# ModelCloud/GPTQModel

Hardware: NVIDIA H100
Metric: W4A16 g128 QuantLinear: decode tok/s + prefill TFLOPS vs HBM/TC roofline (higher is better)
Workload: dtype f16

## Files before the change

### gptqmodel_b200/csrc/b2q_common.cuh

```cuda
#pragma once
#include <cuda_fp16.h>
#include <cuda_bf16.h>
#include <cuda_runtime.h>
#include <stdint.h>

namespace b2q {

__device__ __forceinline__ uint32_t smem_u32(const void* p) {
  return static_cast<uint32_t>(__cvta_generic_to_shared(p));
}

__device__ __forceinline__ uint4 ldg_nc_v4(const void* p) {
  uint4 r;
  asm volatile("ld.global.nc.L1::no_allocate.v4.u32 {%0,%1,%2,%3}, [%4];"
               : "=r"(r.x), "=r"(r.y), "=r"(r.z), "=r"(r.w)
               : "l"(p));
  return r;
}

__device__ __forceinline__ uint32_t lop3_and_or(uint32_t a, uint32_t mask, uint32_t orv) {
  uint32_t r;
  asm("lop3.b32 %0, %1, %2, %3, 0xEA;" : "=r"(r) : "r"(a), "r"(mask), "r"(orv));
  return r;
}

__device__ __forceinline__ float fhfma_lo(uint32_t a2, uint32_t b2, float c) {
  return fmaf(__low2float(*reinterpret_cast<const __half2*>(&a2)), __low2float(*reinterpret_cast<const __half2*>(&b2)), c);
}
__device__ __forceinline__ float fhfma_hi(uint32_t a2, uint32_t b2, float c) {
  return fmaf(__high2float(*reinterpret_cast<const __half2*>(&a2)), __high2float(*reinterpret_cast<const __half2*>(&b2)),
              c);
}
__device__ __forceinline__ float fbfma_lo(uint32_t a2, uint32_t b2, float c) {
  return fmaf(__uint_as_float(a2 << 16), __uint_as_float(b2 << 16), c);
}
__device__ __forceinline__ float fbfma_hi(uint32_t a2, uint32_t b2, float c) {
  return fmaf(__uint_as_float(a2 & 0xFFFF0000u), __uint_as_float(b2 & 0xFFFF0000u), c);
}

__device__ __forceinline__ void mbar_init(uint32_t bar, uint32_t count) {
  asm volatile("mbarrier.init.shared::cta.b64 [%0], %1;" ::"r"(bar), "r"(count));
}
__device__ __forceinline__ void mbar_expect_tx(uint32_t bar, uint32_t bytes) {
  asm volatile("mbarrier.arrive.expect_tx.shared::cta.b64 _, [%0], %1;" ::"r"(bar), "r"(bytes) : "memory");
}
__device__ __forceinline__ void mbar_expect_tx_only(uint32_t bar, uint32_t bytes) {
  asm volatile("mbarrier.expect_tx.relaxed.cta.shared::cta.b64 [%0], %1;" ::"r"(bar), "r"(bytes) : "memory");
}
__device__ __forceinline__ void mbar_arrive(uint32_t bar) {
  asm volatile("mbarrier.arrive.shared::cta.b64 _, [%0];" ::"r"(bar) : "memory");
}
__device__ __forceinline__ bool mbar_try_wait(uint32_t bar, uint32_t parity) {
  uint32_t ok;
  asm volatile(
      "{ .reg .pred p; mbarrier.try_wait.parity.shared::cta.b64 p, [%1], %2; selp.u32 %0, 1, 0, p; }"
      : "=r"(ok)
      : "r"(bar), "r"(parity)
      : "memory");
  return ok != 0;
}
__device__ __forceinline__ void mbar_wait(uint32_t bar, uint32_t parity) {
  while (!mbar_try_wait(bar, parity)) {
  }
}
__device__ __forceinline__ void fence_mbar_init() {
  asm volatile("fence.mbarrier_init.release.cluster;" ::: "memory");
}
__device__ __forceinline__ void fence_proxy_async_smem() {
  asm volatile("fence.proxy.async.shared::cta;" ::: "memory");
}

__device__ __forceinline__ void tma_load_2d(uint32_t dst, const void* tmap, uint32_t bar, int c0, int c1) {
  asm volatile(
      "cp.async.bulk.tensor.2d.shared::cluster.global.mbarrier::complete_tx::bytes [%0], [%1, {%3, %4}], [%2];"
      ::"r"(dst), "l"(tmap), "r"(bar), "r"(c0), "r"(c1)
      : "memory");
}
__device__ __forceinline__ void bulk_load(uint32_t dst, const void* src, uint32_t bytes, uint32_t bar) {
  asm volatile(
      "cp.async.bulk.shared::cluster.global.mbarrier::complete_tx::bytes [%0], [%1], %2, [%3];"
      ::"r"(dst), "l"(src), "r"(bytes), "r"(bar)
      : "memory");
}
__device__ __forceinline__ void prefetch_tmap(const void* tmap) {
  asm volatile("prefetch.tensormap [%0];" ::"l"(tmap) : "memory");
}

constexpr unsigned long long B2Q_PEER_TIMEOUT_NS = 2000000000ull;
__device__ __forceinline__ bool spin_until_geq_sys(const uint32_t* p, uint32_t target) {
  unsigned long long t0 = 0;
  for (unsigned it = 0;; ++it) {
    uint32_t v;
    asm volatile("ld.acquire.sys.global.u32 %0, [%1];" : "=r"(v) : "l"(p) : "memory");
    if ((int32_t)(v - target) >= 0) return true;
    if ((it & 1023u) == 1023u) {
      unsigned long long now;
      asm volatile("mov.u64 %0, %%globaltimer;" : "=l"(now));
      if (t0 == 0) t0 = now;
      else if (now - t0 > B2Q_PEER_TIMEOUT_NS) return false;
    }
  }
}

__device__ __forceinline__ uint32_t cluster_ctarank() {
  uint32_t r;
  asm volatile("mov.u32 %0, %%cluster_ctarank;" : "=r"(r));
  return r;
}
__device__ __forceinline__ uint32_t cluster_nctarank() {
  uint32_t r;
  asm volatile("mov.u32 %0, %%cluster_nctarank;" : "=r"(r));
  return r;
}
__device__ __forceinline__ void cluster_sync_all() {
  asm volatile("barrier.cluster.arrive.release.aligned;\n\tbarrier.cluster.wait.acquire.aligned;" ::: "memory");
}
__device__ __forceinline__ float ld_dsmem_f32(uint32_t local_saddr, uint32_t cta) {
  uint32_t ra;
  float v;
  asm volatile("mapa.shared::cluster.u32 %0, %1, %2;" : "=r"(ra) : "r"(local_saddr), "r"(cta));
  asm volatile("ld.shared::cluster.f32 %0, [%1];" : "=f"(v) : "r"(ra) : "memory");
  return v;
}
__device__ __forceinline__ void ld_dsmem_v4(uint32_t cluster_saddr, float (&v)[4]) {
  asm volatile("ld.shared::cluster.v4.f32 {%0,%1,%2,%3}, [%4];"
               : "=f"(v[0]), "=f"(v[1]), "=f"(v[2]), "=f"(v[3])
               : "r"(cluster_saddr)
               : "memory");
}
__device__ __forceinline__ void ld_dsmem_v4(uint32_t cluster_saddr, int (&v)[4]) {
  asm volatile("ld.shared::cluster.v4.s32 {%0,%1,%2,%3}, [%4];"
               : "=r"(v[0]), "=r"(v[1]), "=r"(v[2]), "=r"(v[3])
               : "r"(cluster_saddr)
               : "memory");
}
template <int NCH, bool FROM_ZERO, typename V>
__device__ __forceinline__ void dsmem_sum4(uint32_t local, uint32_t stride, uint32_t nrank, V (&a)[NCH][4]) {
  if (FROM_ZERO) {
#pragma unroll
    for (int c = 0; c < NCH; ++c)
#pragma unroll
      for (int i = 0; i < 4; ++i) a[c][i] = V(0);
  }
  for (uint32_t r = 0; r < nrank; ++r) {
    uint32_t ra;
    asm volatile("mapa.shared::cluster.u32 %0, %1, %2;" : "=r"(ra) : "r"(local), "r"(r));
#pragma unroll
    for (int c = 0; c < NCH; ++c) {
      V v[4];
      ld_dsmem_v4(ra + c * stride, v);
#pragma unroll
      for (int i = 0; i < 4; ++i) a[c][i] = (FROM_ZERO || r != 0) ? a[c][i] + v[i] : v[i];
    }
  }
}

template <typename T>
struct ET;
template <>
struct ET<__half> {
  static constexpr int FMT = 0;
  static constexpr uint32_t MAGIC = 0x64006400u;
  static constexpr float LO_BASE = 1024.f;
  static constexpr float HI_BASE = 64.f;
  static constexpr float HI_SCALE = 0.0625f;
  __device__ static __forceinline__ void unpack_w4(uint32_t w, uint32_t (&h)[4]) {
    h[0] = lop3_and_or(w, 0x000f000fu, MAGIC);
    h[1] = lop3_and_or(w, 0x00f000f0u, MAGIC);
    const uint32_t w8 = w >> 8;
    h[2] = lop3_and_or(w8, 0x000f000fu, MAGIC);
    h[3] = lop3_and_or(w8, 0x00f000f0u, MAGIC);
  }
  __device__ static __forceinline__ float to_f(__half v) { return __half2float(v); }
  __device__ static __forceinline__ __half from_f(float v) { return __float2half_rn(v); }
  __device__ static __forceinline__ float fma_lo(uint32_t a, uint32_t b, float c) { return fhfma_lo(a, b, c); }
  __device__ static __forceinline__ float fma_hi(uint32_t a, uint32_t b, float c) { return fhfma_hi(a, b, c); }
  __device__ static __forceinline__ uint32_t pack2(float a, float b) {
    __half2 h = __floats2half2_rn(a, b);
    return *reinterpret_cast<uint32_t*>(&h);
  }
};
template <>
struct ET<__nv_bfloat16> {
  static constexpr int FMT = 1;
  static constexpr uint32_t MAGIC = 0x43004300u;
  static constexpr float LO_BASE = 128.f;
  static constexpr float HI_BASE = 128.f;
  static constexpr float HI_SCALE = 1.0f;
  __device__ static __forceinline__ void unpack_w4(uint32_t w, uint32_t (&h)[4]) {
    h[0] = lop3_and_or(w, 0x000f000fu, MAGIC);
    h[1] = lop3_and_or(w >> 4, 0x000f000fu, MAGIC);
    h[2] = lop3_and_or(w >> 8, 0x000f000fu, MAGIC);
    h[3] = lop3_and_or(w >> 12, 0x000f000fu, MAGIC);
  }
  __device__ static __forceinline__ float to_f(__nv_bfloat16 v) { return __bfloat162float(v); }
  __device__ static __forceinline__ __nv_bfloat16 from_f(float v) { return __float2bfloat16_rn(v); }
  __device__ static __forceinline__ float fma_lo(uint32_t a, uint32_t b, float c) { return fbfma_lo(a, b, c); }
  __device__ static __forceinline__ float fma_hi(uint32_t a, uint32_t b, float c) { return fbfma_hi(a, b, c); }
  __device__ static __forceinline__ uint32_t pack2(float a, float b) {
    __nv_bfloat162 h = __floats2bfloat162_rn(a, b);
    return *reinterpret_cast<uint32_t*>(&h);
  }
};

__device__ __forceinline__ uint32_t e4m3x2(float lo, float hi) {
  uint16_t r;
  asm("cvt.rn.satfinite.e4m3x2.f32 %0, %1, %2;" : "=h"(r) : "f"(hi), "f"(lo));
  return r;
}
template <typename T>
__device__ __forceinline__ uint2 fblk_code8(const uint4& v, float s) {
  const T* h = reinterpret_cast<const T*>(&v);
  float q[8];
#pragma unroll
  for (int e = 0; e < 8; ++e) q[e] = ET<T>::to_f(h[e]) / s;
  return make_uint2(e4m3x2(q[0], q[1]) | (e4m3x2(q[2], q[3]) << 16), e4m3x2(q[4], q[5]) | (e4m3x2(q[6], q[7]) << 16));
}

}
```

### gptqmodel_b200/csrc/b2q_gemm.cu

```cuda
#include <cuda.h>

#include "b2q_common.cuh"
#include "b2q_dequant.cuh"
#include "b2q_gemm.cuh"
#include "b2q_internal.h"
#include "b2q_wgmma.cuh"

namespace b2q {

template <typename T, int BITS, bool ASYM, int STAGES, bool FP8 = false>
__global__ void __launch_bounds__(G_THREADS, 1)
    gemm_kernel(const __grid_constant__ CUtensorMap tmap_x, const __grid_constant__ GemmSets S, int M, int K,
                int gshc) {
  using C = GemmCfg<BITS, STAGES>;
  using E = ET<T>;
  extern __shared__ uint8_t smem_raw[];
  const uint32_t smem_base = (smem_u32(smem_raw) + 1023u) & ~1023u;
  uint8_t* smem = smem_raw + (smem_base - smem_u32(smem_raw));

  const uint32_t sA = smem_base;
  const uint32_t sB = sA + STAGES * C::A_BYTES;
  const uint32_t sP = sB + STAGES * C::B_BYTES;
  const uint32_t sBar = sP + STAGES * C::P_BYTES;
  const uint32_t bar_full = sBar, bar_bready = sBar + 8 * STAGES, bar_empty = sBar + 16 * STAGES;

  int set = 0, tn = blockIdx.x;
  if (S.nsets > 1 && tn >= S.tn_end[0]) {
    set = (S.nsets > 2 && tn >= S.tn_end[1]) ? 2 : 1;
    tn -= S.tn_end[set - 1];
  }
  const int N = S.N[set];
  const uint4* __restrict__ packed = S.packed[set];
  const T* __restrict__ scales = reinterpret_cast<const T*>(S.scales[set]);
  const uint32_t* __restrict__ qzeros = S.qzeros[set];

  const int warp = threadIdx.x >> 5, lane = threadIdx.x & 31;
  const int NT = N >> 5;
  const int n0 = tn * G_BN, m0 = blockIdx.y * G_BM;
  const int nt0 = n0 >> 5;
  const int ntiles = min(4, NT - nt0);
  const int nkb = K / G_BK;

  if (threadIdx.x == 0) {
    prefetch_tmap(&tmap_x);
    for (int s = 0; s < STAGES; ++s) {
      mbar_init(bar_full + 8 * s, 1);
      mbar_init(bar_bready + 8 * s, G_DQ_THREADS);
      mbar_init(bar_empty + 8 * s, 1);
    }
    fence_mbar_init();
  }
  __syncthreads();

  if (warp == 8) {
    if (lane == 0) {
      const int FT = N >> 4, ft0 = n0 >> 4;
      const uint32_t pbytes4 = (uint32_t)min(8, FT - ft0) * 512u;
      const uint32_t pbytes8 = (uint32_t)ntiles * C::SUB * 512u;
      for (int kb = 0; kb < nkb; ++kb) {
        const int s = kb % STAGES;
        const uint32_t ph = (kb / STAGES) & 1;
        mbar_wait(bar_empty + 8 * s, ph ^ 1);
        const int g0 = (2 * kb) >> gshc, g1 = (2 * kb + 1) >> gshc;
        const int nrows = (g1 != g0) ? 2 : 1;
        const uint32_t sbytes = (uint32_t)min(G_BN, N - n0) * 2u, zbytes = ASYM ? sbytes / 4u : 0u;
        mbar_expect_tx(bar_full + 8 * s,
                       C::A_BYTES + (BITS == 4 ? pbytes4 + nrows * (sbytes + zbytes) : 2 * pbytes8));
        tma_load_2d(sA + s * C::A_BYTES, &tmap_x, bar_full + 8 * s, kb * G_BK, m0);
        if (BITS == 4) {
          bulk_load(sP + s * C::P_BYTES, packed + ((size_t)kb * FT + ft0) * 32, pbytes4, bar_full + 8 * s);
          for (int r = 0; r < nrows; ++r) {
            const int gr = r ? g1 : g0;
            bulk_load(sP + s * C::P_BYTES + 4096 + r * 320, scales + (size_t)gr * N + n0, sbytes, bar_full + 8 * s);
            if (ASYM)
              bulk_load(sP + s * C::P_BYTES + 4096 + r * 320 + 256, qzeros + (size_t)gr * (N >> 3) + (n0 >> 3),
                        zbytes, bar_full + 8 * s);
          }
        } else {
#pragma unroll
          for (int j = 0; j < 2; ++j)
            bulk_load(sP + s * C::P_BYTES + j * C::P_CHUNK_BYTES,
                      packed + ((size_t)(kb * 2 + j) * NT + nt0) * C::SUB * 32, pbytes8, bar_full + 8 * s);
        }
      }
    }
  } else if (warp < 4) {
    float acc[2][G_BN / 2];
#pragma unroll
    for (int mb = 0; mb < 2; ++mb)
#pragma unroll
      for (int i = 0; i < G_BN / 2; ++i) acc[mb][i] = 0.f;
    for (int kb = 0; kb < nkb; ++kb) {
      const int s = kb % STAGES;
      const uint32_t ph = (kb / STAGES) & 1;
      mbar_wait(bar_full + 8 * s, ph);
      mbar_wait(bar_bready + 8 * s, ph);
      wgmma_fence();
      const uint64_t bdesc = wgmma_desc_k_sw128(sB + s * C::B_BYTES);
      const uint64_t adesc = wgmma_desc_k_sw128(sA + s * C::A_BYTES);
#pragma unroll
      for (int k = 0; k < G_BK / 16; ++k) {
#pragma unroll
        for (int mb = 0; mb < 2; ++mb)
          Wgmma<E::FMT, G_BN>::mma(acc[mb], adesc + 512 * mb + 2 * k, bdesc + 2 * k, (kb | k) != 0 ? 1u : 0u);
      }
      wgmma_commit();
      wgmma_wait<1>();
      if (kb > 0 && threadIdx.x == 0) mbar_arrive(bar_empty + 8 * ((kb - 1) % STAGES));
    }
    wgmma_wait<0>();
#pragma unroll
    for (int mb = 0; mb < 2; ++mb) wgmma_fence_regs(acc[mb]);

    const T* __restrict__ bias = reinterpret_cast<const T*>(S.bias[set]);
    T* __restrict__ out = reinterpret_cast<T*>(S.out[set]);
#pragma unroll
    for (int mb = 0; mb < 2; ++mb) {
#pragma unroll
      for (int h = 0; h < 2; ++h) {
        const int row = m0 + 64 * mb + 16 * warp + (lane >> 2) + 8 * h;
        if (row >= M) continue;
        T* dst = out + (size_t)row * N;
#pragma unroll
        for (int j = 0; j < G_BN / 8; ++j) {
          const int col = n0 + 8 * j + 2 * (lane & 3);
          if (col >= N) continue;
          float f0 = acc[mb][4 * j + 2 * h], f1 = acc[mb][4 * j + 2 * h + 1];
          if (bias != nullptr) {
            f0 = E::to_f(E::from_f(f0)) + E::to_f(bias[col]);
            f1 = E::to_f(E::from_f(f1)) + E::to_f(bias[col + 1]);
          }
          *reinterpret_cast<uint32_t*>(dst + col) = E::pack2(f0, f1);
        }
      }
    }
  } else {
    const int t = threadIdx.x - G_MMA_THREADS;
    constexpr int PF = 32 / BITS;
    constexpr int ZSYM = 1 << (BITS - 1);
    if (BITS == 4) {
      const int lp = t & 31, g = lp >> 2, tt = lp & 3;
      int f[4];
      f[0] = (t >> 5) * 16 + g;
      f[1] = f[0] + 8;
      f[2] = f[0] + 64;
      f[3] = f[0] + 72;
      for (int kb = 0; kb < nkb; ++kb) {
        const int s = kb % STAGES;
        const uint32_t ph = (kb / STAGES) & 1;
        mbar_wait(bar_full + 8 * s, ph);
        const uint8_t* pst = smem + (sP - smem_base) + s * C::P_BYTES;
        const uint4* pj = reinterpret_cast<const uint4*>(pst);
        const int grow = ((2 * kb + (tt >> 1)) >> gshc) - ((2 * kb) >> gshc);
        const uint8_t* srow = pst + 4096 + grow * 320;
#pragma unroll
        for (int u = 0; u < 2; ++u) {
          const uint4 pv = pj[t + u * 128];
          const uint32_t s_lo = *reinterpret_cast<const uint16_t*>(srow + f[2 * u] * 2);
          const uint32_t s_hi = *reinterpret_cast<const uint16_t*>(srow + f[2 * u + 1] * 2);
          int zl = ZSYM, zh = ZSYM;
          if (ASYM) {
            const uint32_t zwl = *reinterpret_cast<const uint32_t*>(srow + 256 + (f[2 * u] >> 3) * 4);
            const uint32_t zwh = *reinterpret_cast<const uint32_t*>(srow + 256 + (f[2 * u + 1] >> 3) * 4);
            zl = (int)((zwl >> (4 * g)) & 15u);
            zh = (int)((zwh >> (4 * g)) & 15u);
          }
          uint4 lo[2], hi[2];
          Dequant<T, 4>::run(pv, s_lo, zl, s_hi, zh, lo, hi);
          const uint32_t sw = (uint32_t)g;
          const uint32_t rlo = sB + s * C::B_BYTES + f[2 * u] * 128;
          const uint32_t rhi = rlo + 8 * 128;
#pragma unroll
          for (int c = 0; c < 2; ++c) {
            const uint32_t off = (((uint32_t)(2 * tt + c)) ^ sw) << 4;
            asm volatile("st.shared.v4.u32 [%0], {%1,%2,%3,%4};" ::"r"(rlo + off), "r"(lo[c].x), "r"(lo[c].y),
                         "r"(lo[c].z), "r"(lo[c].w)
                         : "memory");
            asm volatile("st.shared.v4.u32 [%0], {%1,%2,%3,%4};" ::"r"(rhi + off), "r"(hi[c].x), "r"(hi[c].y),
                         "r"(hi[c].z), "r"(hi[c].w)
                         : "memory");
          }
        }
        fence_proxy_async_smem();
        mbar_arrive(bar_bready + 8 * s);
      }
    } else {
      const int n = n0 + t;
      const int nsafe = (n < N) ? n : 0;
      const int ntl = t >> 5;
      SZRaw cur[2], nxt[2];
      cur[0] = load_sz<T, BITS, ASYM>(scales, qzeros, 0, nsafe, N);
      cur[1] = load_sz<T, BITS, ASYM>(scales, qzeros, 1 >> gshc, nsafe, N);
      for (int kb = 0; kb < nkb; ++kb) {
        const int s = kb % STAGES;
        const uint32_t ph = (kb / STAGES) & 1;
        if (kb + 1 < nkb) {
          nxt[0] = load_sz<T, BITS, ASYM>(scales, qzeros, (2 * kb + 2) >> gshc, nsafe, N);
          nxt[1] = load_sz<T, BITS, ASYM>(scales, qzeros, (2 * kb + 3) >> gshc, nsafe, N);
        }
        mbar_wait(bar_full + 8 * s, ph);
        const uint32_t brow = sB + s * C::B_BYTES + t * 128;
        const uint32_t sw = (uint32_t)(t & 7);
#pragma unroll
        for (int j = 0; j < 2; ++j) {
          int z = ZSYM;
          if (ASYM) z = (int)((cur[j].zw >> (BITS * (nsafe % PF))) & ((1u << BITS) - 1));
          Fp8Div dv = {};
          if constexpr (FP8) dv = fp8_div_of<T>(cur[j].s);
          const uint4* pj = reinterpret_cast<const uint4*>(smem + (sP - smem_base) + s * C::P_BYTES +
                                                           j * C::P_CHUNK_BYTES);
#pragma unroll
          for (int h = 0; h < 2; ++h) {
            const uint4 pv = pj[(ntl * 2 + h) * 32 + lane];
            uint4 o[2];
            if constexpr (FP8)
              DequantFp8<T>::run(pv, dv, o);
            else
              Dequant<T, 8>::run(pv, cur[j].s, z, o);
#pragma unroll
            for (int c = 0; c < 2; ++c) {
              const uint32_t addr = brow + (((uint32_t)(j * 4 + h * 2 + c) ^ sw) << 4);
              asm volatile("st.shared.v4.u32 [%0], {%1,%2,%3,%4};" ::"r"(addr), "r"(o[c].x), "r"(o[c].y),
                           "r"(o[c].z), "r"(o[c].w)
                           : "memory");
            }
          }
        }
        fence_proxy_async_smem();
        mbar_arrive(bar_bready + 8 * s);
        cur[0] = nxt[0];
        cur[1] = nxt[1];
      }
    }
  }
}

typedef CUresult (*EncodeTiledFn)(CUtensorMap*, CUtensorMapDataType, cuuint32_t, void*, const cuuint64_t*,
                                  const cuuint64_t*, const cuuint32_t*, const cuuint32_t*, CUtensorMapInterleave,
                                  CUtensorMapSwizzle, CUtensorMapL2promotion, CUtensorMapFloatOOBfill);

int make_tmap_2d(CUtensorMap* map, CUtensorMapDataType dt, const void* p, int dim0, int dim1, size_t stride, int box0,
                 int box1, CUtensorMapSwizzle sw) {
  struct Entry {
    const void* p;
    int dt, dim0, dim1, box0, box1, sw;
    size_t stride;
    CUtensorMap map;
  };
  constexpr int NCACHE = 64;
  static thread_local Entry cache[NCACHE];
  static thread_local int next = 0, filled = 0;
  for (int i = 0; i < filled; ++i) {
    const Entry& c = cache[i];
    if (c.p == p && c.dt == (int)dt && c.dim0 == dim0 && c.dim1 == dim1 && c.stride == stride && c.box0 == box0 &&
        c.box1 == box1 && c.sw == (int)sw) {
      *map = c.map;
      return 0;
    }
  }
  static EncodeTiledFn enc = nullptr;
  if (enc == nullptr) {
    void* f = nullptr;
    cudaDriverEntryPointQueryResult qres;
    if (cudaGetDriverEntryPoint("cuTensorMapEncodeTiled", &f, cudaEnableDefault, &qres) == cudaSuccess &&
        qres == cudaDriverEntryPointSuccess)
      enc = reinterpret_cast<EncodeTiledFn>(f);
  }
  if (enc == nullptr) {
    set_error("b2q: cuTensorMapEncodeTiled not available from the driver");
    return -1;
  }
  cuuint64_t gdim[2] = {(cuuint64_t)dim0, (cuuint64_t)dim1};
  cuuint64_t gstride[1] = {(cuuint64_t)stride};
  cuuint32_t boxd[2] = {(cuuint32_t)box0, (cuuint32_t)box1};
  cuuint32_t estr[2] = {1, 1};
  CUresult r = enc(map, dt, 2, const_cast<void*>(p), gdim, gstride, boxd, estr, CU_TENSOR_MAP_INTERLEAVE_NONE, sw,
                   CU_TENSOR_MAP_L2_PROMOTION_L2_256B, CU_TENSOR_MAP_FLOAT_OOB_FILL_NONE);
  if (r != CUDA_SUCCESS) {
    set_error("b2q: cuTensorMapEncodeTiled failed (%d) for %p [%d, %d] box [%d, %d]", (int)r, p, dim1, dim0, box1, box0);
    return -1;
  }
  cache[next] = {p, (int)dt, dim0, dim1, box0, box1, (int)sw, stride, *map};
  next = (next + 1) % NCACHE;
  if (filled < NCACHE) ++filled;
  return 0;
}

int gemm_gshc(const MmArgs& a) {
  if (a.group_size == 32) return 0;
  if (a.group_size == 64) return 1;
  if (a.group_size == 128) return 2;
  return 31;
}


template <typename T, int BITS, bool ASYM, int STAGES, bool FP8 = false>
static int launch_gemm_t(const MmArgs& a, const void* x, const GemmSets& S) {
  using C = GemmCfg<BITS, STAGES>;
  CUtensorMap tmap;
  if (make_tmap_2d(&tmap, a.dtype == 0 ? CU_TENSOR_MAP_DATA_TYPE_FLOAT16 : CU_TENSOR_MAP_DATA_TYPE_BFLOAT16, x, a.K, a.M,
                   (size_t)a.K * 2, G_BK, G_BM, CU_TENSOR_MAP_SWIZZLE_128B) != 0)
    return -1;
  auto kern = gemm_kernel<T, BITS, ASYM, STAGES, FP8>;
  static int smem_opted[32] = {};
  if (int e = ensure_dyn_smem(kern, C::SMEM_BYTES, smem_opted, "b2q_gemm")) return e;
  dim3 grid(S.tn_end[S.nsets - 1], (a.M + G_BM - 1) / G_BM, 1);
  kern<<<grid, G_THREADS, C::SMEM_BYTES, a.stream>>>(tmap, S, a.M, a.K, gemm_gshc(a));
  return (int)cudaGetLastError();
}

static int launch_gemm_sets(const MmArgs& a, const void* x, const GemmSets& S) {
  if (a.fp8) return a.dtype == 0 ? launch_gemm_t<__half, 8, false, 4, true>(a, x, S)
                                 : launch_gemm_t<__nv_bfloat16, 8, false, 4, true>(a, x, S);
  const bool asym = S.qzeros[0] != nullptr;
#define B2Q_GEMM_CASE(T, BITS, ST) \
  (asym ? launch_gemm_t<T, BITS, true, ST>(a, x, S) : launch_gemm_t<T, BITS, false, ST>(a, x, S))
  if (a.dtype == 0) return a.bits == 4 ? B2Q_GEMM_CASE(__half, 4, 4) : B2Q_GEMM_CASE(__half, 8, 4);
  return a.bits == 4 ? B2Q_GEMM_CASE(__nv_bfloat16, 4, 4) : B2Q_GEMM_CASE(__nv_bfloat16, 8, 4);
#undef B2Q_GEMM_CASE
}

int launch_gemm_multi(const MmArgs& a, const void* x, int nsets, const void* const* packed, const void* const* scales,
                      const int32_t* const* qzeros, const void* const* bias, void* const* out, const int* Ns) {
  GemmSets S = {};
  S.nsets = nsets;
  int tn = 0;
  for (int i = 0; i < nsets; ++i) {
    tn += (Ns[i] + G_BN - 1) / G_BN;
    S.tn_end[i] = tn;
    S.N[i] = Ns[i];
    S.packed[i] = (const uint4*)packed[i];
    S.scales[i] = scales[i];
    S.qzeros[i] = (const uint32_t*)qzeros[i];
    S.bias[i] = bias[i];
    S.out[i] = out[i];
  }
  for (int i = nsets; i < G_MAX_SETS; ++i) S.tn_end[i] = tn;
  return launch_gemm_sets(a, x, S);
}

int launch_gemm(const MmArgs& a) {
  if (a.K % G_BK != 0) {
    set_error("b2q_gemm: K=%d must be a multiple of %d", a.K, G_BK);
    return -1;
  }
  const void* x = a.x;
  if (a.perm != nullptr) {
    const size_t need = (size_t)a.M * a.K * 2;
    if (a.workspace == nullptr || a.workspace_bytes < need) {
      set_error("b2q_gemm: act-order needs a %zu-byte workspace (got %zu)", need, a.workspace_bytes);
      return -1;
    }
    int e = launch_permute_cols(a.x, a.perm, a.workspace, a.M, a.K, a.stream);
    if (e != 0) return e;
    x = a.workspace;
  }
  if (a.M <= 128 && env().midm && midm_supported(a)) return launch_midm(a, x);
  const void* packed = a.packed;
  const void* scales = a.scales;
  const int32_t* qzeros = (const int32_t*)a.qzeros;
  const void* bias = a.bias;
  void* out = a.out;
  return launch_gemm_multi(a, x, 1, &packed, &scales, &qzeros, &bias, &out, &a.N);
}

}
```

### gptqmodel_b200/csrc/b2q_gemm.cuh

```cuda
#pragma once
#include "b2q_common.cuh"

namespace b2q {

constexpr int G_BM = 128;
constexpr int G_BN = 128;
constexpr int G_BK = 64;
constexpr int G_MMA_THREADS = 128;
constexpr int G_DQ_THREADS = 128;
constexpr int G_THREADS = G_MMA_THREADS + G_DQ_THREADS + 32;

template <int BITS, int STAGES>
struct GemmCfg {
  static constexpr int SUB = BITS / 4;
  static constexpr int A_BYTES = G_BM * G_BK * 2;
  static constexpr int B_BYTES = G_BN * G_BK * 2;
  static constexpr int P_CHUNK_BYTES = 4 * SUB * 512;
  static constexpr int P_BYTES = 2 * P_CHUNK_BYTES + (BITS == 4 ? 1024 : 0);
  static constexpr int STAGE_BYTES = A_BYTES + B_BYTES + P_BYTES;
  static constexpr int BAR_BYTES = 256;
  static constexpr int SMEM_BYTES = STAGES * STAGE_BYTES + BAR_BYTES + 1024;
  static_assert(SMEM_BYTES <= 227 * 1024, "dynamic shared memory of one CTA");
};

constexpr int G_MAX_SETS = 3;
struct GemmSets {
  int nsets;
  int tn_end[G_MAX_SETS];
  int N[G_MAX_SETS];
  const uint4* packed[G_MAX_SETS];
  const void* scales[G_MAX_SETS];
  const uint32_t* qzeros[G_MAX_SETS];
  const void* bias[G_MAX_SETS];
  void* out[G_MAX_SETS];
};

}
```

Before: 677.3.

## Use two MMA warpgroups per CTA, fold producer into dequant warps, stage epilogue via smem

Raises the GEMM M tile from 128 to 256 with two wgmma warpgroups sharing each dequantized B tile, so the dequant work is amortized over twice the rows. The dedicated TMA producer warp is removed. The first dequant warp now issues loads opportunistically inside wait_full, using test_wait polling on the empty barriers. The epilogue writes accumulators to swizzled shared memory, reusing the A buffers, and then does coalesced 16-byte global stores with bias. This risks more register and smem pressure, fewer CTAs for small M, and producer stalls coupled to dequant progress.

```diff
diff --git a/gptqmodel_b200/csrc/b2q_common.cuh b/gptqmodel_b200/csrc/b2q_common.cuh
--- a/gptqmodel_b200/csrc/b2q_common.cuh
+++ b/gptqmodel_b200/csrc/b2q_common.cuh
@@ -54,6 +54,15 @@
   uint32_t ok;
   asm volatile(
       "{ .reg .pred p; mbarrier.try_wait.parity.shared::cta.b64 p, [%1], %2; selp.u32 %0, 1, 0, p; }"
+      : "=r"(ok)
+      : "r"(bar), "r"(parity)
+      : "memory");
+  return ok != 0;
+}
+__device__ __forceinline__ bool mbar_test_wait(uint32_t bar, uint32_t parity) {
+  uint32_t ok;
+  asm volatile(
+      "{ .reg .pred p; mbarrier.test_wait.parity.shared::cta.b64 p, [%1], %2; selp.u32 %0, 1, 0, p; }"
       : "=r"(ok)
       : "r"(bar), "r"(parity)
       : "memory");
diff --git a/gptqmodel_b200/csrc/b2q_gemm.cu b/gptqmodel_b200/csrc/b2q_gemm.cu
--- a/gptqmodel_b200/csrc/b2q_gemm.cu
+++ b/gptqmodel_b200/csrc/b2q_gemm.cu
@@ -46,45 +46,14 @@
     for (int s = 0; s < STAGES; ++s) {
       mbar_init(bar_full + 8 * s, 1);
       mbar_init(bar_bready + 8 * s, G_DQ_THREADS);
-      mbar_init(bar_empty + 8 * s, 1);
+      mbar_init(bar_empty + 8 * s, G_MMA_WGS);
     }
     fence_mbar_init();
   }
   __syncthreads();
 
-  if (warp == 8) {
-    if (lane == 0) {
-      const int FT = N >> 4, ft0 = n0 >> 4;
-      const uint32_t pbytes4 = (uint32_t)min(8, FT - ft0) * 512u;
-      const uint32_t pbytes8 = (uint32_t)ntiles * C::SUB * 512u;
-      for (int kb = 0; kb < nkb; ++kb) {
-        const int s = kb % STAGES;
-        const uint32_t ph = (kb / STAGES) & 1;
-        mbar_wait(bar_empty + 8 * s, ph ^ 1);
-        const int g0 = (2 * kb) >> gshc, g1 = (2 * kb + 1) >> gshc;
-        const int nrows = (g1 != g0) ? 2 : 1;
-        const uint32_t sbytes = (uint32_t)min(G_BN, N - n0) * 2u, zbytes = ASYM ? sbytes / 4u : 0u;
-        mbar_expect_tx(bar_full + 8 * s,
-                       C::A_BYTES + (BITS == 4 ? pbytes4 + nrows * (sbytes + zbytes) : 2 * pbytes8));
-        tma_load_2d(sA + s * C::A_BYTES, &tmap_x, bar_full + 8 * s, kb * G_BK, m0);
-        if (BITS == 4) {
-          bulk_load(sP + s * C::P_BYTES, packed + ((size_t)kb * FT + ft0) * 32, pbytes4, bar_full + 8 * s);
-          for (int r = 0; r < nrows; ++r) {
-            const int gr = r ? g1 : g0;
-            bulk_load(sP + s * C::P_BYTES + 4096 + r * 320, scales + (size_t)gr * N + n0, sbytes, bar_full + 8 * s);
-            if (ASYM)
-              bulk_load(sP + s * C::P_BYTES + 4096 + r * 320 + 256, qzeros + (size_t)gr * (N >> 3) + (n0 >> 3),
-                        zbytes, bar_full + 8 * s);
-          }
-        } else {
-#pragma unroll
-          for (int j = 0; j < 2; ++j)
-            bulk_load(sP + s * C::P_BYTES + j * C::P_CHUNK_BYTES,
-                      packed + ((size_t)(kb * 2 + j) * NT + nt0) * C::SUB * 32, pbytes8, bar_full + 8 * s);
-        }
-      }
-    }
-  } else if (warp < 4) {
+  if (threadIdx.x < G_MMA_THREADS) {
+    const int wg = threadIdx.x >> 7, tw = threadIdx.x & 127;
     float acc[2][G_BN / 2];
 #pragma unroll
     for (int mb = 0; mb < 2; ++mb)
@@ -97,7 +66,7 @@
       mbar_wait(bar_bready + 8 * s, ph);
       wgmma_fence();
       const uint64_t bdesc = wgmma_desc_k_sw128(sB + s * C::B_BYTES);
-      const uint64_t adesc = wgmma_desc_k_sw128(sA + s * C::A_BYTES);
+      const uint64_t adesc = wgmma_desc_k_sw128(sA + s * C::A_BYTES + wg * 128 * 128);
 #pragma unroll
       for (int k = 0; k < G_BK / 16; ++k) {
 #pragma unroll
@@ -106,38 +75,101 @@
       }
       wgmma_commit();
       wgmma_wait<1>();
-      if (kb > 0 && threadIdx.x == 0) mbar_arrive(bar_empty + 8 * ((kb - 1) % STAGES));
+      if (kb > 0 && tw == 0) mbar_arrive(bar_empty + 8 * ((kb - 1) % STAGES));
     }
     wgmma_wait<0>();
 #pragma unroll
     for (int mb = 0; mb < 2; ++mb) wgmma_fence_regs(acc[mb]);
 
+    asm volatile("bar.sync 1, %0;" ::"r"(G_MMA_THREADS) : "memory");
+    const uint32_t stile = sA + wg * (128 * G_BN * 2);
+    const int wq = warp & 3;
+#pragma unroll
+    for (int mb = 0; mb < 2; ++mb)
+#pragma unroll
+      for (int h = 0; h < 2; ++h) {
+        const int r = 64 * mb + 16 * wq + (lane >> 2) + 8 * h;
+#pragma unroll
+        for (int j = 0; j < G_BN / 8; ++j) {
+          const uint32_t addr = stile + r * (G_BN * 2) + ((uint32_t)(j ^ (lane >> 2)) << 4) + 4 * (lane & 3);
+          const uint32_t v = E::pack2(acc[mb][4 * j + 2 * h], acc[mb][4 * j + 2 * h + 1]);
+          asm volatile("st.shared.u32 [%0], %1;" ::"r"(addr), "r"(v) : "memory");
+        }
+      }
+    asm volatile("bar.sync %0, 128;" ::"r"(2 + wg) : "memory");
     const T* __restrict__ bias = reinterpret_cast<const T*>(S.bias[set]);
     T* __restrict__ out = reinterpret_cast<T*>(S.out[set]);
-#pragma unroll
-    for (int mb = 0; mb < 2; ++mb) {
-#pragma unroll
-      for (int h = 0; h < 2; ++h) {
-        const int row = m0 + 64 * mb + 16 * warp + (lane >> 2) + 8 * h;
-        if (row >= M) continue;
-        T* dst = out + (size_t)row * N;
-#pragma unroll
-        for (int j = 0; j < G_BN / 8; ++j) {
-          const int col = n0 + 8 * j + 2 * (lane & 3);
-          if (col >= N) continue;
-          float f0 = acc[mb][4 * j + 2 * h], f1 = acc[mb][4 * j + 2 * h + 1];
-          if (bias != nullptr) {
-            f0 = E::to_f(E::from_f(f0)) + E::to_f(bias[col]);
-            f1 = E::to_f(E::from_f(f1)) + E::to_f(bias[col + 1]);
-          }
-          *reinterpret_cast<uint32_t*>(dst + col) = E::pack2(f0, f1);
-        }
-      }
+#pragma unroll 4
+    for (int i = tw; i < 128 * (G_BN / 8); i += 128) {
+      const int r = i / (G_BN / 8), c = i % (G_BN / 8);
+      const int row = m0 + 128 * wg + r, col = n0 + 8 * c;
+      if (row >= M || col >= N) continue;
+      uint4 v;
+      asm volatile("ld.shared.v4.u32 {%0,%1,%2,%3}, [%4];"
+                   : "=r"(v.x), "=r"(v.y), "=r"(v.z), "=r"(v.w)
+                   : "r"(stile + r * (G_BN * 2) + ((uint32_t)(c ^ (r & 7)) << 4))
+                   : "memory");
+      if (bias != nullptr) {
+        const T* vt = reinterpret_cast<const T*>(&v);
+        uint32_t o[4];
+#pragma unroll
+        for (int e = 0; e < 4; ++e)
+          o[e] = E::pack2(E::to_f(vt[2 * e]) + E::to_f(bias[col + 2 * e]),
+                          E::to_f(vt[2 * e + 1]) + E::to_f(bias[col + 2 * e + 1]));
+        v = make_uint4(o[0], o[1], o[2], o[3]);
+      }
+      *reinterpret_cast<uint4*>(out + (size_t)row * N + col) = v;
     }
   } else {
     const int t = threadIdx.x - G_MMA_THREADS;
     constexpr int PF = 32 / BITS;
     constexpr int ZSYM = 1 << (BITS - 1);
+
+    int kl = 0;
+    auto load_block = [&](int kb) {
+      const int s = kb % STAGES;
+      const int FT = N >> 4, ft0 = n0 >> 4;
+      const uint32_t pbytes4 = (uint32_t)min(8, FT - ft0) * 512u;
+      const uint32_t pbytes8 = (uint32_t)ntiles * C::SUB * 512u;
+      const int g0 = (2 * kb) >> gshc, g1 = (2 * kb + 1) >> gshc;
+      const int nrows = (g1 != g0) ? 2 : 1;
+      const uint32_t sbytes = (uint32_t)min(G_BN, N - n0) * 2u, zbytes = ASYM ? sbytes / 4u : 0u;
+      mbar_expect_tx(bar_full + 8 * s, C::A_BYTES + (BITS == 4 ? pbytes4 + nrows * (sbytes + zbytes) : 2 * pbytes8));
+      tma_load_2d(sA + s * C::A_BYTES, &tmap_x, bar_full + 8 * s, kb * G_BK, m0);
+      if (BITS == 4) {
+        bulk_load(sP + s * C::P_BYTES, packed + ((size_t)kb * FT + ft0) * 32, pbytes4, bar_full + 8 * s);
+        for (int r = 0; r < nrows; ++r) {
+          const int gr = r ? g1 : g0;
+          bulk_load(sP + s * C::P_BYTES + 4096 + r * 320, scales + (size_t)gr * N + n0, sbytes, bar_full + 8 * s);
+          if (ASYM)
+            bulk_load(sP + s * C::P_BYTES + 4096 + r * 320 + 256, qzeros + (size_t)gr * (N >> 3) + (n0 >> 3), zbytes,
+                      bar_full + 8 * s);
+        }
+      } else {
+#pragma unroll
+        for (int j = 0; j < 2; ++j)
+          bulk_load(sP + s * C::P_BYTES + j * C::P_CHUNK_BYTES, packed + ((size_t)(kb * 2 + j) * NT + nt0) * C::SUB * 32,
+                    pbytes8, bar_full + 8 * s);
+      }
+    };
+    auto wait_full = [&](int kb) {
+      const uint32_t bar = bar_full + 8 * (kb % STAGES), ph = (kb / STAGES) & 1;
+      if (t < 32) {
+        while (kl < nkb && kl < kb + STAGES) {
+          const uint32_t e = bar_empty + 8 * (kl % STAGES), eph = ((kl / STAGES) & 1) ^ 1;
+          if (kl <= kb)
+            mbar_wait(e, eph);
+          else if (!__all_sync(0xffffffffu, mbar_test_wait(e, eph))) {
+            if (__all_sync(0xffffffffu, mbar_test_wait(bar, ph))) return;
+            continue;
+          }
+          if (lane == 0) load_block(kl);
+          ++kl;
+        }
+      }
+      mbar_wait(bar, ph);
+    };
+
     if (BITS == 4) {
       const int lp = t & 31, g = lp >> 2, tt = lp & 3;
       int f[4];
@@ -147,8 +179,7 @@
       f[3] = f[0] + 72;
       for (int kb = 0; kb < nkb; ++kb) {
         const int s = kb % STAGES;
-        const uint32_t ph = (kb / STAGES) & 1;
-        mbar_wait(bar_full + 8 * s, ph);
+        wait_full(kb);
         const uint8_t* pst = smem + (sP - smem_base) + s * C::P_BYTES;
         const uint4* pj = reinterpret_cast<const uint4*>(pst);
         const int grow = ((2 * kb + (tt >> 1)) >> gshc) - ((2 * kb) >> gshc);
@@ -193,12 +224,11 @@
       cur[1] = load_sz<T, BITS, ASYM>(scales, qzeros, 1 >> gshc, nsafe, N);
       for (int kb = 0; kb < nkb; ++kb) {
         const int s = kb % STAGES;
-        const uint32_t ph = (kb / STAGES) & 1;
         if (kb + 1 < nkb) {
           nxt[0] = load_sz<T, BITS, ASYM>(scales, qzeros, (2 * kb + 2) >> gshc, nsafe, N);
           nxt[1] = load_sz<T, BITS, ASYM>(scales, qzeros, (2 * kb + 3) >> gshc, nsafe, N);
         }
-        mbar_wait(bar_full + 8 * s, ph);
+        wait_full(kb);
         const uint32_t brow = sB + s * C::B_BYTES + t * 128;
         const uint32_t sw = (uint32_t)(t & 7);
 #pragma unroll
diff --git a/gptqmodel_b200/csrc/b2q_gemm.cuh b/gptqmodel_b200/csrc/b2q_gemm.cuh
--- a/gptqmodel_b200/csrc/b2q_gemm.cuh
+++ b/gptqmodel_b200/csrc/b2q_gemm.cuh
@@ -3,12 +3,13 @@
 
 namespace b2q {
 
-constexpr int G_BM = 128;
+constexpr int G_BM = 256;
 constexpr int G_BN = 128;
 constexpr int G_BK = 64;
-constexpr int G_MMA_THREADS = 128;
+constexpr int G_MMA_WGS = 2;
+constexpr int G_MMA_THREADS = 128 * G_MMA_WGS;
 constexpr int G_DQ_THREADS = 128;
-constexpr int G_THREADS = G_MMA_THREADS + G_DQ_THREADS + 32;
+constexpr int G_THREADS = G_MMA_THREADS + G_DQ_THREADS;
 
 template <int BITS, int STAGES>
 struct GemmCfg {
@@ -21,6 +22,7 @@
   static constexpr int BAR_BYTES = 256;
   static constexpr int SMEM_BYTES = STAGES * STAGE_BYTES + BAR_BYTES + 1024;
   static_assert(SMEM_BYTES <= 227 * 1024, "dynamic shared memory of one CTA");
+  static_assert(STAGES * A_BYTES >= G_MMA_WGS * 128 * G_BN * 2, "epilogue staging");
 };
 
 constexpr int G_MAX_SETS = 3;
```

Result: no change. 677.5 (median of 6 runs) (+0.0%).
